# CycloneBoy/pdf_table

Measured on AMD Instinct MI355X. Metric: pages/s, higher is better.
Workload: dtype bf16

## Files before the change

### include/pdftable_hip.h

```cpp
#ifndef PDFTABLE_HIP_H
#define PDFTABLE_HIP_H

#include <stddef.h>
#include <stdint.h>

#ifdef __cplusplus
extern "C" {
#endif

#define PT_OK 0
#define PT_ERR_INVALID 1
#define PT_ERR_HIP 2
#define PT_ERR_STATE 3
#define PT_ERR_FORMAT 4

typedef struct pt_engine pt_engine;
typedef void* pt_stream;

int pt_engine_create(int device_id, pt_engine** out);
void pt_engine_destroy(pt_engine* e);
const char* pt_last_error(void);
int pt_abi_version(void);
int pt_engine_check(pt_engine* e);
int pt_engine_set_lstm_cluster(pt_engine* e, int on);
// ... 122 lines not shown
  int32_t img_w;
  int32_t reserved;
  int64_t out_off;
} pt_rec_pp_item;
int pt_rec_pp_preprocess(pt_engine* e, const uint8_t* d_pages_rgb, int n_pages, int h, int w, const pt_rec_line* d_lines,
                         const int64_t* h_crop_px, int n_lines, const pt_rec_pp_item* d_items, int n_items, int img_h,
                         int max_img_w, float* d_out, pt_stream stream);
int pt_rec_pp_preprocess_crops(pt_engine* e, const uint8_t* d_crops_rgb, const pt_rec_line* d_lines, const int64_t* h_crop_px,
                               int n_lines, const pt_rec_pp_item* d_items, int n_items, int img_h, int max_img_w, float* d_out,
                               pt_stream stream);

typedef struct pt_tsr_table {
  double minv[6];
  int32_t page, x0, y0, crop_w, crop_h, reserved;
} pt_tsr_table;

int pt_tsr_preprocess(pt_engine* e, const uint8_t* d_pages_rgb, int n_pages, int ph, int pw, const pt_tsr_table* d_tables,
                      int n, int inp_h, int inp_w, int bgr, uint16_t* d_out_bf16, pt_stream stream);

#define PT_TSR_CS_SMALL 8
#define PT_TSR_CS_FEAT 256
int pt_tsr_forward_net(pt_engine* e, const uint16_t* d_input_bf16, int n, int H, int W, float* d_hm, float* d_st,
                       float* d_wh, float* d_ax, float* d_cr, float* d_reg, pt_stream stream);

int pt_tsr_forward_net_wireless(pt_engine* e, const uint16_t* d_input_bf16, int n, int H, int W, float* d_hm, float* d_st,
                                float* d_wh, float* d_ax, float* d_cr, float* d_reg, pt_stream stream);

#define PT_TSR_MAX_CELLS 3000
int pt_tsr_decode(pt_engine* e, const float* d_hm, const float* d_st, const float* d_wh, const float* d_ax,
                  const float* d_cr, const float* d_reg, int n, int h, int w, int wiz_rev, float vis_thresh,
                  int32_t* d_counts, float* d_dets, float* d_logi, pt_stream stream);

int pt_tsr_forward_decode(pt_engine* e, const uint16_t* d_input_bf16, int n, int in_h, int in_w, int wiz_rev,
                          float vis_thresh, int32_t* d_counts, float* d_dets, float* d_logi, pt_stream stream);

int pt_centernet_forward_net(pt_engine* e, const uint16_t* d_input_bf16, int n, int H, int W, float* d_hm, float* d_v2c, float* d_c2v,
                             float* d_reg, pt_stream stream);

#define PT_CENTERNET_MAX_CELLS 1000
int pt_centernet_decode(pt_engine* e, const float* d_hm, const float* d_v2c, const float* d_c2v, const float* d_reg, int n, int h, int w,
                        const double* d_affine, int32_t* d_counts, float* d_cells, pt_stream stream);

int pt_tsr_process(pt_engine* e, const float* d_logi, const float* d_dets, const int32_t* h_counts, int n_tables,
                   int use_2dpe, float* d_logic, float* d_stacked, pt_stream stream);

int pt_op_conv2d(pt_engine* e, const uint16_t* d_in, int B, int H, int W, int Cin, const uint16_t* d_w_tiled,
// ... 98 lines not shown
```

### pdf_table_amd/csrc/api_common.cpp

```cpp
#include <stdarg.h>
#include <stdio.h>

#include "../../include/pdftable_hip.h"

static thread_local char g_err[1024] = "";

void pt_set_error(const char* fmt, ...) {
  va_list ap;
  va_start(ap, fmt);
  vsnprintf(g_err, sizeof(g_err), fmt, ap);
  va_end(ap);
}

extern "C" {

const char* pt_last_error(void) { return g_err; }

int pt_abi_version(void) { return 16; }

}
```

### pdf_table_amd/csrc/c_api.hip

```cpp
#include <stdarg.h>
#include <stdio.h>
#include <stdlib.h>

#include <cmath>

#include "common.h"

namespace PT_FMT_NS {
namespace api {

static int ensure(void** buf, size_t* cap, size_t need);

int pt_engine_check(pt_engine* e) {
  PT_REQUIRE(e, "pt_engine_check: null engine");
  if (e->lstm_err && *e->lstm_err) {
    *e->lstm_err = 0;
    e->lstm_cluster = 0;
    pt_set_error("lstm_cluster_kernel: a workgroup waited > 2^22 polls for its peers -- the launch was not co-resident "
                 "(GPU shared with another process or stream?).  The recognition results since the last check are invalid; "
                 "this engine now uses the streaming LSTM kernel (pt_engine_set_lstm_cluster(e, 0)): run the batch again");
    return PT_ERR_HIP;
  }
  return PT_OK;
}
// ... 313 lines not shown
                      int n, int inp_h, int inp_w, int bgr, uint16_t* d_out_bf16, pt_stream stream) {
  PT_REQUIRE(e && d_pages_rgb && d_tables && d_out_bf16 && n > 0 && n_pages > 0, "pt_tsr_preprocess: bad arguments");
  PT_HIP_CHECK(hipSetDevice(e->device));
  if (!e->tsr_lut) {
    const float mean[3] = {0.408f, 0.447f, 0.470f}, stdv[3] = {0.289f, 0.274f, 0.278f};
    float lut[768];
    for (int c = 0; c < 3; ++c)
      for (int v = 0; v < 256; ++v) lut[c * 256 + v] = (float)(((double)v / 255.0 - (double)mean[c]) / (double)stdv[c]);
    PT_HIP_CHECK(hipMalloc(reinterpret_cast<void**>(&e->tsr_lut), sizeof(lut)));
    PT_HIP_CHECK(hipMemcpy(e->tsr_lut, lut, sizeof(lut), hipMemcpyHostToDevice));
  }
  return pt_launch_tsr_preprocess(d_pages_rgb, ph, pw, d_tables, n, inp_h, inp_w, bgr, e->tsr_lut, d_out_bf16,
                                  pt_split(e), reinterpret_cast<hipStream_t>(stream));
}

int pt_tsr_forward_net(pt_engine* e, const uint16_t* d_input_bf16, int n, int H, int W, float* d_hm, float* d_st,
                       float* d_wh, float* d_ax, float* d_cr, float* d_reg, pt_stream stream) {
  PT_REQUIRE(e && d_input_bf16 && n > 0, "pt_tsr_forward_net: bad arguments");
  PT_HIP_CHECK(hipSetDevice(e->device));
  return pt_lore_forward_net(e, d_input_bf16, n, H, W, d_hm, d_st, d_wh, d_ax, d_cr, d_reg,
                             reinterpret_cast<hipStream_t>(stream));
}

int pt_tsr_forward_net_wireless(pt_engine* e, const uint16_t* d_input_bf16, int n, int H, int W, float* d_hm, float* d_st,
                                float* d_wh, float* d_ax, float* d_cr, float* d_reg, pt_stream stream) {
  PT_REQUIRE(e && d_input_bf16 && n > 0, "pt_tsr_forward_net_wireless: bad arguments");
  PT_HIP_CHECK(hipSetDevice(e->device));
  return pt_lore_wireless_forward_net(e, d_input_bf16, n, H, W, d_hm, d_st, d_wh, d_ax, d_cr, d_reg,
                                      reinterpret_cast<hipStream_t>(stream));
}

int pt_tsr_decode(pt_engine* e, const float* d_hm, const float* d_st, const float* d_wh, const float* d_ax,
                  const float* d_cr, const float* d_reg, int n, int h, int w, int wiz_rev, float vis_thresh,
                  int32_t* d_counts, float* d_dets, float* d_logi, pt_stream stream) {
  PT_REQUIRE(e && n > 0 && h > 0 && w > 0, "pt_tsr_decode: bad arguments");
  PT_HIP_CHECK(hipSetDevice(e->device));
  return pt_lore_decode(e, d_hm, d_st, d_wh, d_ax, d_cr, d_reg, n, h, w, wiz_rev, vis_thresh, d_counts, d_dets, d_logi,
                        reinterpret_cast<hipStream_t>(stream));
}

int pt_centernet_forward_net(pt_engine* e, const uint16_t* d_input_bf16, int n, int H, int W, float* d_hm, float* d_v2c, float* d_c2v,
                             float* d_reg, pt_stream stream) {
  PT_REQUIRE(e && d_input_bf16 && n > 0, "pt_centernet_forward_net: bad arguments");
  PT_HIP_CHECK(hipSetDevice(e->device));
  return pt_centernet_net(e, d_input_bf16, n, H, W, d_hm, d_v2c, d_c2v, d_reg, reinterpret_cast<hipStream_t>(stream));
}
// ... 683 lines not shown
```

### pdf_table_amd/csrc/common.h

```cpp
#pragma once
#include <hip/hip_runtime.h>
#include <stdint.h>
#include <string.h>

#include <map>
#include <string>
#include <vector>

#include "../../include/pdftable_hip.h"
#include "act16.h"

typedef uint16_t bf16_t;

void pt_set_error(const char* fmt, ...);

#define PT_HIP_CHECK(expr)                                                                  \
  do {                                                                                      \
    hipError_t _e = (expr);                                                                 \
    if (_e != hipSuccess) {                                                                 \
      pt_set_error("%s failed: %s (%s:%d)", #expr, hipGetErrorString(_e), __FILE__, __LINE__); \
      return PT_ERR_HIP;                                                                    \
    }                                                                                       \
  } while (0)

// ... 326 lines not shown
                              int* counts, hipStream_t s);
int pt_lore_decode(pt_engine* e, const float* hm, const float* st, const float* wh, const float* ax, const float* cr,
                   const float* reg, int B, int H, int W, int wiz_rev, float vis_thresh, int* d_counts, float* d_dets,
                   float* d_logi, hipStream_t s);
void pt_lore_mosaic_rows(int B, int* rows_ax, int* rows_cr, int* rows_cell, int* rows_corner);
int pt_lore_decode_peaks(pt_engine* e, const float* hm, int B, int H, int W, int wiz_rev, float vis_thresh, int* d_counts,
                         const int** d_lim_cell, const int** d_lim_corner, hipStream_t s);
int pt_lore_peak_patches(pt_engine* e, const bf16_t* feat, int B, int H, int W, int C, int split, bf16_t* mos_cell,
                         bf16_t* mos_corner, hipStream_t s);
int pt_lore_decode_boxes(pt_engine* e, const float* reg_cell, const float* wh, const float* reg_corner, const float* st, int B,
                         int H, int W, const int** d_lim_ax, const int** d_lim_cr, hipStream_t s);
int pt_lore_patch_gather(pt_engine* e, const bf16_t* feat, int B, int H, int W, int C, int split, bf16_t* mos_ax, bf16_t* mos_cr,
                         hipStream_t s);
int pt_lore_decode_sparse(pt_engine* e, const float* ax_mos, const float* cr_mos, int B, int H, int W, float vis_thresh,
                          int* d_counts, float* d_dets, float* d_logi, hipStream_t s);
int pt_lore_forward_decode(pt_engine* e, const bf16_t* x, int n, int H, int W, int wiz_rev, float vis_thresh, int* d_counts,
                           float* d_dets, float* d_logi, hipStream_t s);
int pt_lore_wireless_forward_net(pt_engine* e, const bf16_t* x, int n, int H, int W, float* hm, float* st, float* wh,
                                 float* ax, float* cr, float* reg, hipStream_t s);
int pt_lore_process(pt_engine* e, const float* d_logi, const float* d_dets, const int32_t* h_counts, int n_tables,
                    int use_2dpe, float* d_logic, float* d_stacked, hipStream_t s);
int pt_lore_forward_net(pt_engine* e, const bf16_t* x, int n, int H, int W, float* hm, float* st, float* wh, float* ax,
                        float* cr, float* reg, hipStream_t s);
constexpr int PT_HEAT_CAP = 16384;
int pt_heat_peaks_topk(const float* hm, int B, int H, int W, float thr0, float thr1, int k0, int k1, float* sig, unsigned long long* keys,
                       int* cnt, unsigned long long* sorted, int* kept, hipStream_t s);
int pt_centernet_net(pt_engine* e, const bf16_t* x, int n, int H, int W, float* hm, float* v2c, float* c2v, float* reg, hipStream_t s);
int pt_centernet_decode_maps(pt_engine* e, const float* hm, const float* v2c, const float* c2v, const float* reg, int B, int H, int W,
                             const double* affine, int* d_counts, float* d_cells, hipStream_t s);

static inline int pt_split(const pt_engine* e) { return e->precision == PT_PRECISION_BF16X3 || e->precision == PT_PRECISION_F16X2; }
static inline int pt_f16x2(const pt_engine* e) { return e->precision == PT_PRECISION_F16X2; }

struct PtProfScope {
  pt_engine* e;
  hipStream_t s;
  int idx = -1;
  PtProfScope(pt_engine* e_, hipStream_t s_, int cls, double flop, const char* label = "") : e(e_), s(s_) {
    double bytes = 0;
    if (e) { bytes = e->prof.next_bytes; e->prof.next_bytes = 0; }
    if (e && e->prof.on && (e->prof.on == 1 || e->prof.on - 2 == cls)) {
      PtProfile::Pending p;
      p.bytes = bytes;
      if (hipEventCreate(&p.a) != hipSuccess || hipEventCreate(&p.b) != hipSuccess) return;
      p.cls = cls;
      p.flop = flop;
// ... 23 lines not shown
```

### pdf_table_amd/csrc/dla_net.h

```cpp
#pragma once

#include <stdlib.h>

#include <string>
#include <vector>

#include "common.h"

namespace PT_FMT_NS {

int pt_launch_conv3x3_c16(pt_engine* e, const bf16_t* in, const bf16_t* w, const float* bias, bf16_t* out, int B, int H, int W,
                          int N, int stride, int split, hipStream_t s);
int pt_launch_dla_thin_chain(pt_engine* e, const bf16_t* in, int B, int H, int W, const bf16_t* w_stem, const float* b_stem, const bf16_t* w0,
                             const float* b0, const bf16_t* w1, const float* b1, bf16_t* out, hipStream_t s);

namespace {

struct T {
  bf16_t* p = nullptr;
  int H = 0, W = 0, C = 0;
};

struct DlaCtx {
  pt_engine* e;
  const PtModel* m;
  const char* what = "Lore DLA-34";
  hipStream_t s;
  int n, x3, mul;
  bool dry;
  bool ok;
  int rc;
  bf16_t* cols = nullptr;
  float* om = nullptr;
  const int* ylimit = nullptr;
  double alg_scale = 1.0;

  T alloc(int H, int W, int C) {
    T t;
    t.H = H; t.W = W; t.C = C;
    t.p = reinterpret_cast<bf16_t*>(e->arenas[PT_ARENA_TSR].take((size_t)n * H * W * C * mul * sizeof(bf16_t)));
    if (!t.p) ok = false;
    return t;
  }
  const PtTensor* get(const std::string& name) {
    const PtTensor* t = m->find(name);
    if (!t && rc == PT_OK) {
      pt_set_error("%s weight blob lacks tensor '%s'", what, name.c_str());
      rc = PT_ERR_FORMAT;
    }
    return t;
  }
  void conv(const T& in, const std::string& q, int N, int ks, int stride, const T& out, int relu, const T* res = nullptr,
            int nv = 0, float* out_f32 = nullptr, int f32_cs = 0, int cin_override = 0, int alg_n = 0) {
    const PtTensor* w = get(q + (x3 ? ".w3" : ".w"));
    const PtTensor* b = get(q + ".b");
    if (rc != PT_OK || dry || !ok) return;
    ConvDesc c;
    c.in = in.p; c.B = n; c.H = in.H; c.W = in.W; c.Cin = cin_override ? cin_override : in.C;
    c.w = reinterpret_cast<const bf16_t*>(w->d_ptr); c.bias = reinterpret_cast<const float*>(b->d_ptr);
    c.N = N; c.ks = ks; c.stride = stride; c.relu = relu; c.split = x3; c.n_valid = nv; c.ylimit = ylimit;
    c.alg_n = alg_n; c.alg_scale = alg_scale;
    if (out_f32) {
      c.out_f32 = out_f32; c.out_cstride = f32_cs;
    } else {
      c.out = out.p; c.out_cstride = out.C * mul; c.out_lo_off = out.C;
    }
    if (res) { c.res = res->p; c.res_mode = 1; }
// ... 1 lines not shown
    if (r != PT_OK) rc = r;
  }
  void conv_cat(const std::vector<T>& ins, const std::string& q, int N, const T& out, int relu) {
    const PtTensor* w = get(q + (x3 ? ".w3" : ".w"));
    const PtTensor* b = get(q + ".b");
    if (rc != PT_OK || dry || !ok) return;
    ConvDesc c;
    c.in = ins[0].p; c.B = n; c.H = ins[0].H; c.W = ins[0].W;
    c.nseg = (int)ins.size();
    c.Cin = 0;
    for (int i = 0; i < c.nseg; ++i) {
      c.seg_c[i] = ins[i].C;
      c.Cin += ins[i].C;
      if (i) c.in_more[i - 1] = ins[i].p;
    }
    c.w = reinterpret_cast<const bf16_t*>(w->d_ptr); c.bias = reinterpret_cast<const float*>(b->d_ptr);
    c.N = N; c.ks = 1; c.stride = 1; c.relu = relu; c.split = x3; c.alg_scale = alg_scale;
    c.out = out.p; c.out_cstride = out.C * mul; c.out_lo_off = out.C;
    const int r = pt_launch_conv(e, c, s);
    if (r != PT_OK) rc = r;
  }
  T maxpool2(const T& x) {
    T o = alloc(x.H / 2, x.W / 2, x.C);
    if (rc == PT_OK && !dry && ok) {
      e->prof.next_bytes = (double)n * x.H * x.W * x.C * 2.0 * mul * 1.25;
      PtProfScope ps(e, s, PT_PROF_OTHER, 0, "maxpool2x2");
      const int r = pt_launch_maxpool_kxk(x.p, n, x.H, x.W, x.C, 2, 2, 0, x3, o.p, s);
      if (r != PT_OK) rc = r;
    }
    return o;
  }
  T block(const std::string& q, const T& x, const T& residual, int stride, int cout) {
    T t = alloc(x.H / stride, x.W / stride, cout);
    conv(x, q + ".conv1", cout, 3, stride, t, 1);
    T o = alloc(t.H, t.W, cout);
    conv(t, q + ".conv2", cout, 3, 1, o, 1, &residual);
    return o;
  }
  T tree(const std::string& q, int levels, const T& x, int cin, int cout, int stride, bool level_root,
         std::vector<T> children) {
    T bottom = stride > 1 ? maxpool2(x) : x;
    if (level_root) children.push_back(bottom);
    if (levels == 1) {
      T residual = bottom;
      if (cin != cout) {
        residual = alloc(bottom.H, bottom.W, cout);
        conv(bottom, q + ".project", cout, 1, 1, residual, 0);
      }
      T x1 = block(q + ".tree1", x, residual, stride, cout);
      T x2 = block(q + ".tree2", x1, x1, 1, cout);
      std::vector<T> ins = {x2, x1};
      ins.insert(ins.end(), children.begin(), children.end());
      T o = alloc(x1.H, x1.W, cout);
      conv_cat(ins, q + ".root", cout, o, 1);
      return o;
    }
    T x1 = tree(q + ".tree1", levels - 1, x, cin, cout, stride, false, {});
    children.push_back(x1);
    return tree(q + ".tree2", levels - 1, x1, cout, cout, 1, false, children);
  }
};

static std::vector<T> dla34_base(DlaCtx& c, const bf16_t* x, int H, int W) {
  pt_engine* e = c.e;
  hipStream_t s = c.s;
  const int n = c.n;
  const int ch[6] = {16, 32, 64, 128, 256, 512};
  const int lv[6] = {1, 1, 1, 2, 2, 1};
  const char* chain_env = getenv("PT_DLA_CHAIN");
  const bool chain = !c.x3 && H % 2 == 0 && W % 2 == 0 && !(chain_env && atoi(chain_env) == 0);
  std::vector<T> layers(6);
  if (chain) {
    layers[1] = c.alloc(H / 2, W / 2, 32);
    const PtTensor *ws = c.get("base_layer.w"), *bs = c.get("base_layer.b"), *w0 = c.get("level0.wt"), *b0 = c.get("level0.bt"),
                   *w1 = c.get("level1.wt"), *b1 = c.get("level1.bt");
    if (c.rc == PT_OK && !c.dry && c.ok) {
      const int r = pt_launch_dla_thin_chain(e, x, n, H, W, reinterpret_cast<const bf16_t*>(ws->d_ptr), reinterpret_cast<const float*>(bs->d_ptr),
                                             reinterpret_cast<const bf16_t*>(w0->d_ptr), reinterpret_cast<const float*>(b0->d_ptr),
                                             reinterpret_cast<const bf16_t*>(w1->d_ptr), reinterpret_cast<const float*>(b1->d_ptr), layers[1].p, s);
      if (r != PT_OK) c.rc = r;
    }
  } else {
    T t0 = c.alloc(H, W, 16);
    if (!c.dry && c.ok) {
      const PtTensor* w = c.get(c.x3 ? "base_layer.w3" : "base_layer.w");
      const PtTensor* b = c.get("base_layer.b");
      if (c.rc == PT_OK) {
        const int r = pt_launch_stem7x7(e, x, n, H, W, reinterpret_cast<const bf16_t*>(w->d_ptr),
                                        reinterpret_cast<const float*>(b->d_ptr), t0.p, c.x3, s, 1, 16);
        if (r != PT_OK) c.rc = r;
      }
    }
    layers[0] = c.alloc(H, W, 16);
    layers[1] = c.alloc(H / 2, W / 2, 32);
    for (int lv1 = 0; lv1 < 2; ++lv1) {
      const std::string q = lv1 ? "level1" : "level0";
      const PtTensor* w = c.get(q + (c.x3 ? ".wt3" : ".wt"));
      const PtTensor* b = c.get(q + ".bt");
      if (c.rc == PT_OK && !c.dry && c.ok) {
        const int r = pt_launch_conv3x3_c16(e, lv1 ? layers[0].p : t0.p, reinterpret_cast<const bf16_t*>(w->d_ptr),
                                            reinterpret_cast<const float*>(b->d_ptr), layers[lv1].p, n, H, W, lv1 ? 32 : 16,
                                            lv1 ? 2 : 1, c.x3, s);
        if (r != PT_OK) c.rc = r;
      }
    }
  }
  for (int l = 2; l < 6; ++l)
    layers[l] = c.tree("level" + std::to_string(l), lv[l], layers[l - 1], ch[l - 1], ch[l], 2, l > 2, {});
  return layers;
}

static int dla_arena_grow(pt_engine* e) {
  PT_HIP_CHECK(hipDeviceSynchronize());
  if (e->arenas[PT_ARENA_TSR].base) PT_HIP_CHECK(hipFree(e->arenas[PT_ARENA_TSR].base));
  e->arenas[PT_ARENA_TSR].base = nullptr;
  const size_t want = pt_arena_round(e->arenas[PT_ARENA_TSR].high);
  PT_HIP_CHECK(hipMalloc(reinterpret_cast<void**>(&e->arenas[PT_ARENA_TSR].base), want));
  e->arenas[PT_ARENA_TSR].cap = want;
  return PT_OK;
}

}

}
```

### pdf_table_amd/csrc/lore_kernels.hip

```cpp
#include <stdio.h>
#include <stdlib.h>

#include "common.h"

namespace PT_FMT_NS {

typedef __attribute__((ext_vector_type(4))) uint32_t u32x4;
typedef __attribute__((ext_vector_type(2))) uint32_t u32x2;

namespace {

__device__ __forceinline__ float bf2f(uint32_t b) { return a16_to_f32(b); }
__device__ __forceinline__ uint32_t f2bf(float f) { return f32_to_a16(f); }

__device__ __forceinline__ void load8(const bf16_t* p, int lo_off, int split, float* v) {
  const u32x4 h = *reinterpret_cast<const u32x4*>(p);
  const uint32_t hw[4] = {h.x, h.y, h.z, h.w};
#pragma unroll
  for (int k = 0; k < 8; ++k) v[k] = bf2f((k & 1) ? (hw[k >> 1] >> 16) : (hw[k >> 1] & 0xFFFFu));
  if (split) {
    const u32x4 l = *reinterpret_cast<const u32x4*>(p + lo_off);
    const uint32_t lw[4] = {l.x, l.y, l.z, l.w};
#pragma unroll
    for (int k = 0; k < 8; ++k) v[k] += bf2f((k & 1) ? (lw[k >> 1] >> 16) : (lw[k >> 1] & 0xFFFFu));
// ... 210 lines not shown
        if (add) {
          float a[8];
          if (PACKED) {
            const uint32_t hw[4] = {araw[py][px].x, araw[py][px].y, araw[py][px].z, araw[py][px].w};
#pragma unroll
            for (int k = 0; k < 8; ++k) a[k] = bf2f((k & 1) ? (hw[k >> 1] >> 16) : (hw[k >> 1] & 0xFFFFu));
            if (SP) {
              const u32x4 rl = alo[SP ? py : 0][SP ? px : 0];
              const uint32_t lw[4] = {rl.x, rl.y, rl.z, rl.w};
#pragma unroll
              for (int k = 0; k < 8; ++k) a[k] += bf2f((k & 1) ? (lw[k >> 1] >> 16) : (lw[k >> 1] & 0xFFFFu));
            }
          } else {
            load8(add + oo, C, split, a);
          }
#pragma unroll
          for (int q = 0; q < 8; ++q) acc[q] += a[q];
        }
        if (SLICE)
          store8(out + (((size_t)b * (2 * h) + 2 * ay + py) * OW + 2 * ax + px) * ocs + cg * 8, olo, PACKED == 1 ? 0 : split, acc);
        else
          store8(out + oo, C, PACKED == 1 ? 0 : split, acc);
      }
  }
}

__global__ __launch_bounds__(256) void tsr_preprocess_kernel(const uint8_t* __restrict__ pages, int ph, int pw,
                                                              const pt_tsr_table* __restrict__ tabs, int H, int W, int bgr,
                                                              const float* __restrict__ lut, bf16_t* __restrict__ out,
                                                              int split) {
  a16_kernel_enter();
  const int t = blockIdx.y;
  const int i = blockIdx.x * blockDim.x + threadIdx.x;
  if (i >= H * W) return;
  const int y = i / W, x = i - y * W;
  const pt_tsr_table tb = tabs[t];
  auto sat = [](double v) { return (long long)fmin(fmax(rint(v), -2147483648.0), 2147483647.0); };
  const long long adelta = sat(tb.minv[0] * x * 1024.0), bdelta = sat(tb.minv[3] * x * 1024.0);
  const long long X0 = sat((tb.minv[1] * y + tb.minv[2]) * 1024.0) + 16, Y0 = sat((tb.minv[4] * y + tb.minv[5]) * 1024.0) + 16;
  const long long X = (X0 + adelta) >> 5, Y = (Y0 + bdelta) >> 5;
  long long sx = X >> 5, sy = Y >> 5;
  sx = sx < -32768 ? -32768 : (sx > 32767 ? 32767 : sx);
  sy = sy < -32768 ? -32768 : (sy > 32767 ? 32767 : sy);
  const int ax = (int)(X & 31), ay = (int)(Y & 31);
  const int wt[4] = {(32 - ay) * (32 - ax) * 32, (32 - ay) * ax * 32, ay * (32 - ax) * 32, ay * ax * 32};
  int acc[3] = {0, 0, 0};
// ... 1403 lines not shown
int pt_launch_dwconvt_up_add(const bf16_t* in, const float* w, const bf16_t* add, bf16_t* out, int B, int h, int wd,
                             int C, int f, int split, hipStream_t s) {
  PT_REQUIRE(in && w && out && C % 8 == 0 && (f == 2 || f == 4), "dwconvT: bad arguments");
  const long long blocks2 = (long long)B * h * wd * (C / 8);
  const char* sw = getenv("PT_DWCONVT2");
  if (f == 2 && blocks2 < (1ll << 31) && C <= 512 && !(sw && sw[0] == '0')) {
    static int packed = -1;
    if (packed < 0) {
      const char* ev = getenv("PT_DWCONVT2_PACKED");
      packed = ev ? atoi(ev) : 1;
    }
    if (!split && packed)
      hipLaunchKernelGGL(dwconvt_up2_add_kernel<1>, dim3(grid_for(blocks2)), dim3(256), (size_t)16 * C * sizeof(float), s, in, w, add, out,
                         B, h, wd, C, 0);
    else if (split && packed)
      hipLaunchKernelGGL(dwconvt_up2_add_kernel<2>, dim3(grid_for(blocks2)), dim3(256), (size_t)16 * C * sizeof(float), s, in, w, add, out,
                         B, h, wd, C, 1);
    else
      hipLaunchKernelGGL(dwconvt_up2_add_kernel<0>, dim3(grid_for(blocks2)), dim3(256), (size_t)16 * C * sizeof(float), s, in, w, add, out,
                         B, h, wd, C, split);
    PT_HIP_CHECK(hipGetLastError());
    return PT_OK;
  }
  hipLaunchKernelGGL(dwconvt_up_add_kernel, dim3(grid_for((long long)B * h * f * wd * f * (C / 8))), dim3(256), 0, s, in,
                     w, add, out, B, h, wd, C, f, split);
  PT_HIP_CHECK(hipGetLastError());
  return PT_OK;
}

int pt_launch_dwconvt_up2_slice(const bf16_t* in, const float* w, bf16_t* out, int out_cstride, int out_coff, int out_lo_off, int B,
                                int h, int wd, int C, int split, hipStream_t s) {
  PT_REQUIRE(in && w && out && C % 8 == 0 && C <= 512 && out_cstride % 8 == 0 && out_coff % 8 == 0 && out_lo_off % 8 == 0 &&
                 out_coff + C * (split ? 2 : 1) <= out_cstride && (!split || out_coff + out_lo_off + C <= out_cstride),
             "dwconvT slice: bad arguments");
  const long long blocks2 = (long long)B * h * wd * (C / 8);
  PT_REQUIRE(blocks2 < (1ll << 31), "dwconvT slice: map too large");
  if (split)
    hipLaunchKernelGGL((dwconvt_up2_add_kernel<2, true>), dim3(grid_for(blocks2)), dim3(256), (size_t)16 * C * sizeof(float), s, in, w,
                       (const bf16_t*)nullptr, out + out_coff, B, h, wd, C, 1, out_cstride, out_lo_off);
  else
    hipLaunchKernelGGL((dwconvt_up2_add_kernel<1, true>), dim3(grid_for(blocks2)), dim3(256), (size_t)16 * C * sizeof(float), s, in, w,
                       (const bf16_t*)nullptr, out + out_coff, B, h, wd, C, 0, out_cstride, 0);
  PT_HIP_CHECK(hipGetLastError());
  return PT_OK;
}

// ... 181 lines not shown
```

### pdf_table_amd/csrc/lore_model.hip

```cpp
#include "dla_net.h"

namespace PT_FMT_NS {

int pt_launch_dcn_im2col(const bf16_t* x, const float* om, bf16_t* cols, int B, int H, int W, int C, int split,
                         hipStream_t s);
int pt_launch_dwconvt_up_add(const bf16_t* in, const float* w, const bf16_t* add, bf16_t* out, int B, int h, int wd,
                             int C, int f, int split, hipStream_t s);

namespace {

struct Ctx : DlaCtx {
  T dcn(const std::string& q, const T& x, int cout) {
    T o = alloc(x.H, x.W, cout);
    static const bool fused = !(getenv("PT_DCN_FUSED") && atoi(getenv("PT_DCN_FUSED")) == 0);
    const bool om_inside = fused && pt_dcn_fuses_om(e, x.C, x3);
    if (!om_inside) conv(x, q + ".om", 64, 3, 1, T(), 0, nullptr, 32, om, 32, 0, 27);
    if (fused) {
      const PtTensor* w = get(q + (x3 ? ".dcn.w3" : ".dcn.w"));
      const PtTensor* b = get(q + ".dcn.b");
      const PtTensor* ow = om_inside ? get(q + (x3 ? ".om.w3" : ".om.w")) : nullptr;
      const PtTensor* ob = om_inside ? get(q + ".om.b") : nullptr;
      if (rc == PT_OK && !dry && ok) {
        const int r = pt_launch_dcn_fused(e, x.p, om, reinterpret_cast<const bf16_t*>(w->d_ptr),
                                          reinterpret_cast<const float*>(b->d_ptr), o.p, n, x.H, x.W, x.C, cout, x3, 1, s,
// ... 144 lines not shown
        head(mcr_, rows_cr, "cr", 256, ocr, lim_cr, 256);
        if (c.rc != PT_OK) return c.rc;
        r = pt_lore_decode_sparse(e, oax, ocr, n, feat.H, feat.W, sp->vis_thresh, sp->d_counts, sp->d_dets, sp->d_logi, s);
        if (r != PT_OK) return r;
      }
    }
    if (c.rc != PT_OK) return c.rc;
    if (pass == 0) {
      if (c.ok) continue;
      const int r = dla_arena_grow(e);
      if (r != PT_OK) return r;
      continue;
    }
    if (!c.ok) {
      pt_set_error("Lore net: activation arena allocation failed");
      return PT_ERR_HIP;
    }
    break;
  }
  return PT_OK;
}


int pt_lore_forward_net(pt_engine* e, const bf16_t* x, int n, int H, int W, float* hm, float* st, float* wh, float* ax,
                        float* cr, float* reg, hipStream_t s) {
  PT_REQUIRE(hm && st && wh && ax && cr && reg, "Lore net: null pointer");
  return lore_dla_run(e, x, n, H, W, hm, st, wh, ax, cr, reg, nullptr, s);
}

int pt_lore_forward_decode(pt_engine* e, const bf16_t* x, int n, int H, int W, int wiz_rev, float vis_thresh, int* d_counts,
                           float* d_dets, float* d_logi, hipStream_t s) {
  PT_REQUIRE(d_counts && d_dets && d_logi, "Lore forward+decode: null pointer");
  SparseArgs sp{wiz_rev, vis_thresh, d_counts, d_dets, d_logi};
  return lore_dla_run(e, x, n, H, W, nullptr, nullptr, nullptr, nullptr, nullptr, nullptr, &sp, s);
}

namespace {

struct WCtx {
  pt_engine* e;
  const PtModel* m;
  hipStream_t s;
  int n, x3, mul;
  bool dry, ok;
  int rc;
  T alloc(int H, int W, int C) {
// ... 139 lines not shown
```

### pdf_table_amd/engine.py

```python
from __future__ import annotations

import contextlib
import ctypes as C
import functools
import threading
from typing import Optional, Sequence, Tuple

import numpy as np
import torch

from . import lib as L

__all__ = ["HipEngine", "REC_LINE_DTYPE", "CLS_IMAGE_DTYPE", "REC_PP_ITEM_DTYPE"]

TSR_TABLE_DTYPE = np.dtype([("minv", "<f8", (6,)), ("page", "<i4"), ("x0", "<i4"), ("y0", "<i4"),
                            ("crop_w", "<i4"), ("crop_h", "<i4"), ("reserved", "<i4")])
CLS_IMAGE_DTYPE = np.dtype([("offset", "<i8"), ("h", "<i4"), ("w", "<i4")])
REC_LINE_DTYPE = np.dtype([("minv", np.float64, (9,)), ("page", np.int32), ("crop_w", np.int32), ("crop_h", np.int32),
                           ("reserved", np.int32)])


REC_PP_ITEM_DTYPE = np.dtype([("line", "<i4"), ("resized_w", "<i4"), ("img_w", "<i4"), ("reserved", "<i4"),
                              ("out_off", "<i8")])

# ... 649 lines not shown
        pad = k // 2
        out = torch.empty((B, (H + 2 * pad - k) // stride + 1, (W + 2 * pad - k) // stride + 1, Cc), dtype=self.act_dtype, device=self._tdev)
        L.check(self.lib.pt_op_dwconv(self._h, _ptr(x), B, H, W, Cc // 2 if split else Cc, _ptr(w_taps), _ptr(bias), k, stride, act, _ptr(out), int(split),
                                      self._stream()), "pt_op_dwconv")
        return out

    def op_add(self, a: torch.Tensor, b: torch.Tensor, split: bool = False) -> torch.Tensor:
        self._chk(a, self.act_dtype, "a")
        self._chk(b, self.act_dtype, "b")
        if a.shape != b.shape:
            raise ValueError(f"op_add: shapes differ: {tuple(a.shape)} vs {tuple(b.shape)}")
        out = torch.empty_like(a)
        L.check(self.lib.pt_op_add(self._h, _ptr(a), _ptr(b), _ptr(out), a.numel() // a.shape[-1], a.shape[-1] // 2 if split else a.shape[-1], int(split),
                                   self._stream()), "pt_op_add")
        return out

    def op_maxpool(self, x: torch.Tensor, k: int, stride: int, pad: int, split: bool = False) -> torch.Tensor:
        self._chk(x, self.act_dtype, "x")
        B, H, W, Cc = x.shape
        out = torch.empty((B, (H + 2 * pad - k) // stride + 1, (W + 2 * pad - k) // stride + 1, Cc), dtype=self.act_dtype, device=self._tdev)
        L.check(self.lib.pt_op_maxpool(self._h, _ptr(x), B, H, W, Cc // 2 if split else Cc, k, stride, pad, _ptr(out), int(split), self._stream()), "pt_op_maxpool")
        return out

    def op_avgpool(self, x: torch.Tensor, k: int, split: bool = False) -> torch.Tensor:
        self._chk(x, self.act_dtype, "x")
        B, H, W, Cc = x.shape
        out = torch.empty((B, H // k, W // k, Cc), dtype=self.act_dtype, device=self._tdev)
        L.check(self.lib.pt_op_avgpool(self._h, _ptr(x), B, H, W, Cc // 2 if split else Cc, k, _ptr(out), int(split), self._stream()), "pt_op_avgpool")
        return out

    def op_chan_mean(self, x: torch.Tensor, split: bool = False) -> torch.Tensor:
        self._chk(x, self.act_dtype, "x")
        B, H, W, Cc = x.shape
        ch = Cc // 2 if split else Cc
        scratch = torch.empty((self.lib.pt_op_chan_mean_scratch_floats(B, ch),), dtype=torch.float32, device=self._tdev)
        out = torch.empty((B, 1, 1, Cc), dtype=self.act_dtype, device=self._tdev)
        L.check(self.lib.pt_op_chan_mean(self._h, _ptr(x), B, H * W, ch, _ptr(scratch), _ptr(out), int(split), self._stream()), "pt_op_chan_mean")
        return out

    def op_scale_channels(self, x: torch.Tensor, gate: torch.Tensor, split: bool = False) -> torch.Tensor:
        self._chk(x, self.act_dtype, "x")
        self._chk(gate, self.act_dtype, "gate")
        B, H, W, Cc = x.shape
        if gate.numel() != B * Cc:
            raise ValueError(f"op_scale_channels: gate {tuple(gate.shape)} does not match [{B}, {Cc}]")
        out = torch.empty_like(x)
# ... 215 lines not shown
```

### pdf_table_amd/lib.py

```python
from __future__ import annotations

import ctypes as C
import os

_HERE = os.path.dirname(os.path.abspath(__file__))
LIB_PATH = os.environ.get("PT_LIB_PATH") or os.path.join(_HERE, "libpdftable_hip.so")

PT_MODEL_DB_RESNET18 = 1
PT_MODEL_CRNN = 2
PT_MODEL_LORE_DLA34 = 3
PT_MODEL_LORE_PROCESSOR = 4
PT_MODEL_PICODET = 5
PT_MODEL_LORE_RESNET18 = 6
PT_MODEL_DB_NAS = 7
PT_MODEL_PPLCNET = 8
PT_MODEL_CONVNEXT_VIT = 16
PT_MODEL_MTL_BACKBONE = 17
PT_MODEL_MTL_DECODER = 18
PT_MODEL_CENTERNET_DLA34 = 19
PT_CVIT_W, PT_CVIT_CHUNK_W, PT_CVIT_CHUNK_STEP, PT_CVIT_T, PT_CVIT_NCLS = 804, 300, 252, 201, 7644
PT_CLS_SLOTS = 4
PT_CLS_MAX_CLASSES = 16
PT_LAYOUT_HEAD_CS, PT_LAYOUT_CAND_FLOATS = 40, 48
PT_DET_PRE_DB_PP = 0
PT_DET_PRE_DB_TORCH = 1
PT_DET_PRE_NONE = 2
PT_PRECISION_BF16 = 0
PT_PRECISION_BF16X3 = 1
PT_PRECISION_F16X2 = 2
PT_PRECISION_F16 = 3
PT_DET_POST_DB_PP = 0
PT_DET_POST_DB_TORCH = 1
PT_TSR_MAX_CELLS = 3000
PT_CENTERNET_MAX_CELLS = 1000
PT_ROTATE_90_CLOCKWISE, PT_ROTATE_180, PT_ROTATE_90_COUNTERCLOCKWISE = 0, 1, 2
PT_REC_H, PT_REC_W, PT_REC_T, PT_REC_NCLS = 32, 640, 160, 7644
PT_PROF_CLASSES = ("conv3x3", "conv1x1", "stem", "other")
EXPECTED_ABI = 16

_lib = None


class PtError(RuntimeError):
    pass


def _proto(lib):
    vp, i, f, sz = C.c_void_p, C.c_int, C.c_float, C.c_size_t
    ip = C.POINTER(C.c_int)
    P = {
        "pt_engine_create": (i, [i, C.POINTER(vp)]),
        "pt_engine_destroy": (None, [vp]),
        "pt_last_error": (C.c_char_p, []),
        "pt_abi_version": (i, []),
        "pt_engine_check": (i, [vp]),
        "pt_engine_set_precision": (i, [vp, i]),
        "pt_engine_set_lstm_cluster": (i, [vp, i]),
        "pt_engine_set_mtl_kv_fp8": (i, [vp, i]),
        "pt_engine_set_dcn_mfma": (i, [vp, i]),
        "pt_weights_load": (i, [vp, i, vp, sz]),
        "pt_weights_load_device": (i, [vp, i, vp, sz, vp]),
# ... 10 lines not shown
        "pt_rec_forward": (i, [vp, vp, i, i, i, vp, vp, i, vp, vp, vp]),
        "pt_rec_forward_crops": (i, [vp, vp, vp, vp, i, vp, vp, vp]),
        "pt_rec_forward_net": (i, [vp, vp, i, vp, vp, vp]),
        "pt_rec_preprocess": (i, [vp, vp, i, i, i, vp, vp, i, vp, vp]),
        "pt_rec_cvit_forward": (i, [vp, vp, i, i, i, vp, vp, vp, i, vp, vp, vp]),
        "pt_rec_cvit_forward_crops": (i, [vp, vp, vp, vp, vp, i, vp, vp, vp]),
        "pt_rec_cvit_forward_net": (i, [vp, vp, i, i, vp, vp, vp, vp]),
        "pt_rec_cvit_preprocess_crops": (i, [vp, vp, vp, vp, i, vp, vp]),
        "pt_tsr_mtl_backbone_net": (i, [vp, vp, i, i, i, vp, vp]),
        "pt_tsr_mtl_preprocess": (i, [vp, vp, i, i, i, vp, i, i, vp, vp]),
        "pt_tsr_mtl_resized_size": (None, [i, i, i, ip, ip]),
        "pt_tsr_mtl_decoder_config": (i, [vp, ip]),
        "pt_tsr_mtl_structure": (i, [vp, vp, i, i, vp, vp, ip, ip, i, vp]),
        "pt_tsr_mtl_cells": (i, [vp, i, vp, vp, vp, ip, i, vp]),
        "pt_rec_pp_preprocess": (i, [vp, vp, i, i, i, vp, vp, i, vp, i, i, i, vp, vp]),
        "pt_rec_pp_preprocess_crops": (i, [vp, vp, vp, vp, i, vp, i, i, i, vp, vp]),
        "pt_layout_plan": (i, [i, i, ip, ip]),
        "pt_layout_preprocess": (i, [vp, vp, i, i, i, i, i, vp, vp]),
        "pt_layout_forward_net": (i, [vp, vp, i, i, i, vp, vp, vp, vp, vp]),
        "pt_layout_candidates": (i, [vp, vp, vp, vp, vp, i, i, i, i, f, i, vp, vp, vp]),
        "pt_layout_forward": (i, [vp, vp, i, i, i, i, i, i, f, i, vp, vp, vp]),
        "pt_tsr_preprocess": (i, [vp, vp, i, i, i, vp, i, i, i, i, vp, vp]),
        "pt_tsr_forward_net": (i, [vp, vp, i, i, i, vp, vp, vp, vp, vp, vp, vp]),
        "pt_tsr_forward_net_wireless": (i, [vp, vp, i, i, i, vp, vp, vp, vp, vp, vp, vp]),
        "pt_tsr_decode": (i, [vp, vp, vp, vp, vp, vp, vp, i, i, i, i, f, vp, vp, vp, vp]),
        "pt_tsr_forward_decode": (i, [vp, vp, i, i, i, i, f, vp, vp, vp, vp]),
        "pt_tsr_process": (i, [vp, vp, vp, vp, i, i, vp, vp, vp]),
        "pt_centernet_forward_net": (i, [vp, vp, i, i, i, vp, vp, vp, vp, vp]),
        "pt_centernet_decode": (i, [vp, vp, vp, vp, vp, i, i, i, vp, vp, vp, vp]),
        "pt_hard_nms": (i, [vp, vp, vp, i, C.c_double, i, vp, vp]),
        "pt_page_line_mask": (i, [vp, i, i, i, vp, vp]),
        "pt_page_line_angles": (i, [vp, i, i, i, i, i, vp, i, vp]),
        "pt_page_warp_cubic": (i, [vp, i, i, i, vp, vp, i, vp, vp]),
        "pt_page_quarter_turn": (i, [vp, i, i, i, i, vp, vp]),
        "pt_page_pre_tables": (i, [vp, vp]),
        "pt_cls_preprocess": (i, [vp, vp, vp, i, i, i, i, i, vp, vp]),
        "pt_cls_forward_net": (i, [vp, i, vp, i, i, i, i, vp, ip, vp]),
        "pt_cls_forward": (i, [vp, i, vp, vp, i, i, i, i, i, i, vp, ip, vp]),
        "pt_cls_forward_lines": (i, [vp, i, vp, i, i, i, vp, vp, i, i, i, i, i, i, vp, ip, vp]),
        "pt_cls_forward_lines_direct": (i, [vp, i, vp, i, i, i, vp, i, i, i, i, i, i, vp, ip, vp]),
        "pt_op_conv2d": (i, [vp, vp, i, i, i, i, vp, vp, i, i, i, vp, i, i, i, i, vp, i, i, i, i, vp]),
        "pt_op_conv1x1_ex": (i, [vp, vp, i, i, i, i, vp, vp, i, vp, vp, i, i, vp, i, vp, vp]),
        "pt_op_dcn": (i, [vp, vp, vp, i, i, i, i, vp, vp, i, vp, i, i, vp]),
        "pt_op_stem7x7": (i, [vp, vp, i, i, i, vp, vp, vp, i, vp]),
        "pt_op_maxpool3x3s2": (i, [vp, vp, i, i, i, i, vp, i, vp]),
        "pt_op_db_head_final": (i, [vp, vp, i, i, i, vp, vp, vp, vp, i, vp]),
# ... 51 lines not shown
```

Before: 811.4.

## Share maxpool across DLA tree levels and add gather-based 4x depthwise transposed conv

In the DLA-34 tree, the stride-2 maxpool of the input is now computed once and passed down to tree1, so the same pooling is not launched twice; an env var can turn this off. It also adds a dedicated kernel for the f=4 depthwise transposed-conv upsample with fused add. Each thread loads a 3x3 input neighborhood once, keeps the taps in LDS, and writes a 4x4 output block, instead of one thread per output pixel re-reading the input. Plan and op entry points are exposed for testing, and the ABI version is bumped.

```diff
diff --git a/include/pdftable_hip.h b/include/pdftable_hip.h
--- a/include/pdftable_hip.h
+++ b/include/pdftable_hip.h
@@ -168,6 +168,11 @@
 #define PT_TSR_CS_FEAT 256
 int pt_tsr_forward_net(pt_engine* e, const uint16_t* d_input_bf16, int n, int H, int W, float* d_hm, float* d_st,
                        float* d_wh, float* d_ax, float* d_cr, float* d_reg, pt_stream stream);
+
+int pt_tsr_dla34_plan(int n, int H, int W, int32_t* pool_launches, long long* arena_bytes);
+
+int pt_op_dwconvt_up_add(pt_engine* e, const uint16_t* d_in, const float* d_w_taps, const uint16_t* d_add, uint16_t* d_out, int B, int h,
+                         int w, int C, int f, int split, pt_stream stream);
 
 int pt_tsr_forward_net_wireless(pt_engine* e, const uint16_t* d_input_bf16, int n, int H, int W, float* d_hm, float* d_st,
                                 float* d_wh, float* d_ax, float* d_cr, float* d_reg, pt_stream stream);
diff --git a/pdf_table_amd/csrc/api_common.cpp b/pdf_table_amd/csrc/api_common.cpp
--- a/pdf_table_amd/csrc/api_common.cpp
+++ b/pdf_table_amd/csrc/api_common.cpp
@@ -16,6 +16,6 @@
 
 const char* pt_last_error(void) { return g_err; }
 
-int pt_abi_version(void) { return 16; }
+int pt_abi_version(void) { return 17; }
 
 }
diff --git a/pdf_table_amd/csrc/c_api.hip b/pdf_table_amd/csrc/c_api.hip
--- a/pdf_table_amd/csrc/c_api.hip
+++ b/pdf_table_amd/csrc/c_api.hip
@@ -359,6 +359,18 @@
                              reinterpret_cast<hipStream_t>(stream));
 }
 
+int pt_tsr_dla34_plan(int n, int H, int W, int32_t* pool_launches, long long* arena_bytes) {
+  return pt_dla34_base_plan(n, H, W, pool_launches, arena_bytes);
+}
+
+int pt_op_dwconvt_up_add(pt_engine* e, const uint16_t* d_in, const float* d_w_taps, const uint16_t* d_add, uint16_t* d_out, int B, int h, int w,
+                         int C, int f, int split, pt_stream stream) {
+  PT_REQUIRE(e && d_in && d_w_taps && d_out && B > 0 && h > 0 && w > 0 && C > 0 && C % 8 == 0 && (f == 2 || f == 4),
+             "pt_op_dwconvt_up_add: B=%d h=%d w=%d C=%d f=%d unsupported (C a multiple of 8, f 2 or 4)", B, h, w, C, f);
+  PT_HIP_CHECK(hipSetDevice(e->device));
+  return pt_launch_dwconvt_up_add(d_in, d_w_taps, d_add, d_out, B, h, w, C, f, split ? 1 : 0, reinterpret_cast<hipStream_t>(stream));
+}
+
 int pt_tsr_forward_net_wireless(pt_engine* e, const uint16_t* d_input_bf16, int n, int H, int W, float* d_hm, float* d_st,
                                 float* d_wh, float* d_ax, float* d_cr, float* d_reg, pt_stream stream) {
   PT_REQUIRE(e && d_input_bf16 && n > 0, "pt_tsr_forward_net_wireless: bad arguments");
diff --git a/pdf_table_amd/csrc/common.h b/pdf_table_amd/csrc/common.h
--- a/pdf_table_amd/csrc/common.h
+++ b/pdf_table_amd/csrc/common.h
@@ -372,6 +372,9 @@
                     int use_2dpe, float* d_logic, float* d_stacked, hipStream_t s);
 int pt_lore_forward_net(pt_engine* e, const bf16_t* x, int n, int H, int W, float* hm, float* st, float* wh, float* ax,
                         float* cr, float* reg, hipStream_t s);
+int pt_dla34_base_plan(int n, int H, int W, int* pool_launches, long long* arena_bytes);
+int pt_launch_dwconvt_up_add(const bf16_t* in, const float* w, const bf16_t* add, bf16_t* out, int B, int h, int wd, int C, int f, int split,
+                             hipStream_t s);
 constexpr int PT_HEAT_CAP = 16384;
 int pt_heat_peaks_topk(const float* hm, int B, int H, int W, float thr0, float thr1, int k0, int k1, float* sig, unsigned long long* keys,
                        int* cnt, unsigned long long* sorted, int* kept, hipStream_t s);
diff --git a/pdf_table_amd/csrc/dla_net.h b/pdf_table_amd/csrc/dla_net.h
--- a/pdf_table_amd/csrc/dla_net.h
+++ b/pdf_table_amd/csrc/dla_net.h
@@ -34,6 +34,9 @@
   float* om = nullptr;
   const int* ylimit = nullptr;
   double alg_scale = 1.0;
+  bool share_pool = true;
+  bool plan_only = false;
+  int n_pool = 0;
 
   T alloc(int H, int W, int C) {
     T t;
@@ -43,6 +46,7 @@
     return t;
   }
   const PtTensor* get(const std::string& name) {
+    if (plan_only) return nullptr;
     const PtTensor* t = m->find(name);
     if (!t && rc == PT_OK) {
       pt_set_error("%s weight blob lacks tensor '%s'", what, name.c_str());
@@ -90,6 +94,7 @@
   }
   T maxpool2(const T& x) {
     T o = alloc(x.H / 2, x.W / 2, x.C);
+    ++n_pool;
     if (rc == PT_OK && !dry && ok) {
       e->prof.next_bytes = (double)n * x.H * x.W * x.C * 2.0 * mul * 1.25;
       PtProfScope ps(e, s, PT_PROF_OTHER, 0, "maxpool2x2");
@@ -106,8 +111,8 @@
     return o;
   }
   T tree(const std::string& q, int levels, const T& x, int cin, int cout, int stride, bool level_root,
-         std::vector<T> children) {
-    T bottom = stride > 1 ? maxpool2(x) : x;
+         std::vector<T> children, const T* pooled = nullptr) {
+    T bottom = stride > 1 ? (pooled ? *pooled : maxpool2(x)) : x;
     if (level_root) children.push_back(bottom);
     if (levels == 1) {
       T residual = bottom;
@@ -123,7 +128,7 @@
       conv_cat(ins, q + ".root", cout, o, 1);
       return o;
     }
-    T x1 = tree(q + ".tree1", levels - 1, x, cin, cout, stride, false, {});
+    T x1 = tree(q + ".tree1", levels - 1, x, cin, cout, stride, false, {}, share_pool && stride > 1 ? &bottom : nullptr);
     children.push_back(x1);
     return tree(q + ".tree2", levels - 1, x1, cout, cout, 1, false, children);
   }
@@ -137,6 +142,9 @@
   const int lv[6] = {1, 1, 1, 2, 2, 1};
   const char* chain_env = getenv("PT_DLA_CHAIN");
   const bool chain = !c.x3 && H % 2 == 0 && W % 2 == 0 && !(chain_env && atoi(chain_env) == 0);
+  const char* share_env = getenv("PT_DLA_POOL_SHARE");
+  c.share_pool = !(share_env && atoi(share_env) == 0);
+  c.n_pool = 0;
   std::vector<T> layers(6);
   if (chain) {
     layers[1] = c.alloc(H / 2, W / 2, 32);
@@ -178,6 +186,16 @@
   return layers;
 }
 
+static void dla34_plan(int n, int H, int W, int* pool_launches, long long* arena_bytes) {
+  pt_engine host;
+  DlaCtx c;
+  c.e = &host; c.m = nullptr; c.s = nullptr; c.n = n; c.x3 = 0; c.mul = 1;
+  c.dry = true; c.ok = true; c.rc = PT_OK; c.plan_only = true;
+  dla34_base(c, nullptr, H, W);
+  if (pool_launches) *pool_launches = c.n_pool;
+  if (arena_bytes) *arena_bytes = (long long)host.arenas[PT_ARENA_TSR].high;
+}
+
 static int dla_arena_grow(pt_engine* e) {
   PT_HIP_CHECK(hipDeviceSynchronize());
   if (e->arenas[PT_ARENA_TSR].base) PT_HIP_CHECK(hipFree(e->arenas[PT_ARENA_TSR].base));
diff --git a/pdf_table_amd/csrc/lore_kernels.hip b/pdf_table_amd/csrc/lore_kernels.hip
--- a/pdf_table_amd/csrc/lore_kernels.hip
+++ b/pdf_table_amd/csrc/lore_kernels.hip
@@ -256,6 +256,74 @@
         else
           store8(out + oo, C, PACKED == 1 ? 0 : split, acc);
       }
+  }
+}
+
+__global__ __launch_bounds__(256) void dwconvt_up4_add_kernel(const bf16_t* __restrict__ in, const float* __restrict__ w,
+                                                               const bf16_t* __restrict__ add, bf16_t* __restrict__ out,
+                                                               int B, int h, int wd, int C) {
+  a16_kernel_enter();
+  extern __shared__ __attribute__((aligned(16))) float s_w[];
+  for (int i = threadIdx.x; i < 64 * C; i += 256) s_w[i] = w[i];
+  __syncthreads();
+  const int cgn = C >> 3;
+  const int OW = wd * 4;
+  const unsigned total = (unsigned)B * h * wd * cgn;
+  for (unsigned i = blockIdx.x * 256u + threadIdx.x; i < total; i += gridDim.x * 256u) {
+    unsigned t = i / (unsigned)cgn;
+    const int cg = (int)(i - t * (unsigned)cgn);
+    const unsigned t2 = t / (unsigned)wd;
+    const int ax = (int)(t - t2 * (unsigned)wd);
+    const int b = (int)(t2 / (unsigned)h);
+    const int ay = (int)(t2 - (unsigned)b * (unsigned)h);
+    u32x4 vraw[3][3];
+#pragma unroll
+    for (int r = 0; r < 3; ++r)
+#pragma unroll
+      for (int c = 0; c < 3; ++c) {
+        const int iy = ay - 1 + r, ix = ax - 1 + c;
+        const bool ok = iy >= 0 && iy < h && ix >= 0 && ix < wd;
+        const int iyc = min(max(iy, 0), h - 1), ixc = min(max(ix, 0), wd - 1);
+        u32x4 rv = *reinterpret_cast<const u32x4*>(in + (((size_t)b * h + iyc) * wd + ixc) * C + cg * 8);
+        const uint32_t m = ok ? 0xFFFFFFFFu : 0u;
+        rv.x &= m; rv.y &= m; rv.z &= m; rv.w &= m;
+        vraw[r][c] = rv;
+      }
+#pragma unroll
+    for (int py = 0; py < 4; ++py) {
+      const size_t orow = (((size_t)b * (4 * h) + 4 * ay + py) * OW + 4 * ax) * C + cg * 8;
+      u32x4 araw[4];
+      if (add) {
+#pragma unroll
+        for (int px = 0; px < 4; ++px) araw[px] = *reinterpret_cast<const u32x4*>(add + orow + (size_t)px * C);
+      }
+#pragma unroll
+      for (int px = 0; px < 4; ++px) {
+        float acc[8];
+#pragma unroll
+        for (int q = 0; q < 8; ++q) acc[q] = 0.f;
+#pragma unroll
+        for (int dy = 0; dy < 2; ++dy) {
+          const int r = 1 + (py >> 1) - dy;
+          const int ky = py + 2 - 4 * ((py >> 1) - dy);
+#pragma unroll
+          for (int dx = 0; dx < 2; ++dx) {
+            const int c = 1 + (px >> 1) - dx;
+            const int kx = px + 2 - 4 * ((px >> 1) - dx);
+            const float* wp = s_w + (ky * 8 + kx) * C + cg * 8;
+            const uint32_t hw[4] = {vraw[r][c].x, vraw[r][c].y, vraw[r][c].z, vraw[r][c].w};
+#pragma unroll
+            for (int q = 0; q < 8; ++q) acc[q] += bf2f((q & 1) ? (hw[q >> 1] >> 16) : (hw[q >> 1] & 0xFFFFu)) * wp[q];
+          }
+        }
+        if (add) {
+          const uint32_t hw[4] = {araw[px].x, araw[px].y, araw[px].z, araw[px].w};
+#pragma unroll
+          for (int q = 0; q < 8; ++q) acc[q] += bf2f((q & 1) ? (hw[q >> 1] >> 16) : (hw[q >> 1] & 0xFFFFu));
+        }
+        store8(out + orow + (size_t)px * C, C, 0, acc);
+      }
+    }
   }
 }
 
@@ -1705,6 +1773,13 @@
     PT_HIP_CHECK(hipGetLastError());
     return PT_OK;
   }
+  const char* sw4 = getenv("PT_DWCONVT4");
+  if (f == 4 && !split && blocks2 < (1ll << 31) && C <= 128 && !(sw4 && sw4[0] == '0')) {
+    hipLaunchKernelGGL(dwconvt_up4_add_kernel, dim3(grid_for(blocks2)), dim3(256), (size_t)64 * C * sizeof(float), s, in, w, add, out, B, h, wd,
+                       C);
+    PT_HIP_CHECK(hipGetLastError());
+    return PT_OK;
+  }
   hipLaunchKernelGGL(dwconvt_up_add_kernel, dim3(grid_for((long long)B * h * f * wd * f * (C / 8))), dim3(256), 0, s, in,
                      w, add, out, B, h, wd, C, f, split);
   PT_HIP_CHECK(hipGetLastError());
diff --git a/pdf_table_amd/csrc/lore_model.hip b/pdf_table_amd/csrc/lore_model.hip
--- a/pdf_table_amd/csrc/lore_model.hip
+++ b/pdf_table_amd/csrc/lore_model.hip
@@ -190,6 +190,12 @@
 }
 
 
+int pt_dla34_base_plan(int n, int H, int W, int* pool_launches, long long* arena_bytes) {
+  PT_REQUIRE(n > 0 && H > 0 && W > 0 && H % 32 == 0 && W % 32 == 0, "DLA-34 plan: n=%d, input %dx%d must be multiples of 32", n, H, W);
+  dla34_plan(n, H, W, pool_launches, arena_bytes);
+  return PT_OK;
+}
+
 int pt_lore_forward_net(pt_engine* e, const bf16_t* x, int n, int H, int W, float* hm, float* st, float* wh, float* ax,
                         float* cr, float* reg, hipStream_t s) {
   PT_REQUIRE(hm && st && wh && ax && cr && reg, "Lore net: null pointer");
diff --git a/pdf_table_amd/engine.py b/pdf_table_amd/engine.py
--- a/pdf_table_amd/engine.py
+++ b/pdf_table_amd/engine.py
@@ -695,6 +695,21 @@
         L.check(self.lib.pt_op_maxpool(self._h, _ptr(x), B, H, W, Cc // 2 if split else Cc, k, stride, pad, _ptr(out), int(split), self._stream()), "pt_op_maxpool")
         return out
 
+    def op_dwconvt_up_add(self, x: torch.Tensor, w_taps: torch.Tensor, f: int, add: torch.Tensor | None = None, split: bool = False) -> torch.Tensor:
+        self._chk(x, self.act_dtype, "x")
+        B, h, w, Cc = x.shape
+        Cv = Cc // 2 if split else Cc
+        if w_taps.dtype != torch.float32 or tuple(w_taps.shape) != (4 * f * f, Cv) or not w_taps.is_contiguous() or not w_taps.is_cuda:
+            raise ValueError(f"op_dwconvt_up_add: w_taps must be a contiguous fp32 device tensor [{4 * f * f}, {Cv}]")
+        if add is not None:
+            self._chk(add, self.act_dtype, "add")
+            if tuple(add.shape) != (B, h * f, w * f, Cc):
+                raise ValueError(f"op_dwconvt_up_add: add must be {(B, h * f, w * f, Cc)}, got {tuple(add.shape)}")
+        out = torch.empty((B, h * f, w * f, Cc), dtype=self.act_dtype, device=self._tdev)
+        L.check(self.lib.pt_op_dwconvt_up_add(self._h, _ptr(x), _ptr(w_taps), _ptr(add) if add is not None else None, _ptr(out), B, h, w, Cv, f,
+                                              int(split), self._stream()), "pt_op_dwconvt_up_add")
+        return out
+
     def op_avgpool(self, x: torch.Tensor, k: int, split: bool = False) -> torch.Tensor:
         self._chk(x, self.act_dtype, "x")
         B, H, W, Cc = x.shape
diff --git a/pdf_table_amd/lib.py b/pdf_table_amd/lib.py
--- a/pdf_table_amd/lib.py
+++ b/pdf_table_amd/lib.py
@@ -36,7 +36,7 @@
 PT_ROTATE_90_CLOCKWISE, PT_ROTATE_180, PT_ROTATE_90_COUNTERCLOCKWISE = 0, 1, 2
 PT_REC_H, PT_REC_W, PT_REC_T, PT_REC_NCLS = 32, 640, 160, 7644
 PT_PROF_CLASSES = ("conv3x3", "conv1x1", "stem", "other")
-EXPECTED_ABI = 16
+EXPECTED_ABI = 17
 
 _lib = None
 
@@ -93,6 +93,8 @@
         "pt_layout_forward": (i, [vp, vp, i, i, i, i, i, i, f, i, vp, vp, vp]),
         "pt_tsr_preprocess": (i, [vp, vp, i, i, i, vp, i, i, i, i, vp, vp]),
         "pt_tsr_forward_net": (i, [vp, vp, i, i, i, vp, vp, vp, vp, vp, vp, vp]),
+        "pt_tsr_dla34_plan": (i, [i, i, i, ip, C.POINTER(C.c_longlong)]),
+        "pt_op_dwconvt_up_add": (i, [vp, vp, vp, vp, vp, i, i, i, i, i, i, vp]),
         "pt_tsr_forward_net_wireless": (i, [vp, vp, i, i, i, vp, vp, vp, vp, vp, vp, vp]),
         "pt_tsr_decode": (i, [vp, vp, vp, vp, vp, vp, vp, i, i, i, i, f, vp, vp, vp, vp]),
         "pt_tsr_forward_decode": (i, [vp, vp, i, i, i, i, f, vp, vp, vp, vp]),
```

New measurement: 809.5. No clear change (-0.2%).
